# pierric/smart-chess-rust

Measured on AMD Instinct MI355X. Metric: MCTS simulations/sec (whole node), self-play rollout=180, at 1/2/4/8 MI355X, higher is better.
Workload: dtype bf16

## Files before the change

### smart-chess-rust_amd/csrc/mcts_types.hpp

```cpp
#pragma once
#include <stdint.h>

#include "chess_rules.hpp"

namespace sc {

constexpr int MAXC = 224;
enum { ST_IDLE = 0, ST_ACTIVE = 1, ST_FINISHED = 2, ST_PENDING = 3 };
enum { TR_FREE = 0, TR_LIVE = 1, TR_DONE = 2 };
enum { SYNTH_HASH = 1, SYNTH_COARSE = 2, SYNTH_UNIFORM = 3 };
enum { LK_NONE = 0, LK_EVAL = 1, LK_TERM_NEW = 2, LK_TERM_CACHED = 3 };
enum { ERR_NONFINITE_UCT = 1, ERR_POOL_OVERFLOW = 2, ERR_BAD_MOVE_INDEX = 4, ERR_DEPTH_OVERFLOW = 8, ERR_HELPER_TIMEOUT = 16, ERR_HANDOFF_TIMEOUT = 32 };

struct GameCtl {
    int32_t status, ply, sim, n_nodes, n_exp;
    int32_t leaf, path_len, leaf_kind, n_legal;
    float leaf_value;
    uint32_t err;
    int32_t trace_slot;
    uint64_t game_id;
    int32_t start_ply;
    int32_t rollout_cur;
};

struct NodeHdr {
    int32_t fc;
    uint16_t nc;
    uint16_t ps;
};

struct TraceHdr {
    int32_t n_steps, has_outcome, termination, winner;
    uint64_t game_id;
    int32_t state, pad;
};

struct Counters {
    unsigned long long next_game, sims_done, nn_evals, plies_done;
    int32_t games_finished, err;
};

struct SpParams {
    int n_slots, rollout, num_steps, temp_switch, with_noise, outcome_gate, evaluator, external_noise;
    int tie_random;
    int trace_hold;
    float rollout_factor;
    uint64_t synth_salt;
    float cpuct, temperature, epsilon;
    uint64_t seed, first_game_id;
    int node_cap, max_depth, hist_cap, tpos_cap, trace_cap, total_games;
    GameCtl* ctl;
    Position* hist;
    Position* tpos;
    int32_t* path;
    int32_t* N;
    float* W;
    float* P;
    float* U;
    uint16_t* MV;
    NodeHdr* H;
    int8_t* boards;
    int32_t* meta;
    uint16_t* legal_mv;
    uint16_t* legal_idx;
    int32_t* n_legal;
    float* prior;
    float* value;
    float* noise;
    TraceHdr* thdr;
    uint16_t* t_move;
    float* t_q;
    int32_t* t_nchild;
    uint16_t* t_cmove;
    int32_t* t_cn;
    float* t_cq;
    float* t_cu;
    Counters* cnt;
    unsigned long long* slot_cnt;
    int vf_fused, vf_ksplit;
    const float* vpart;
    const float* vf_w;
    uint32_t vf_fc1b, vf_fc1m, vf_fc2w, vf_fc2b;
    const float* choice_w;
    int choice_w_max;
    unsigned long long* dbg_cycles;
};


}
```

### smart-chess-rust_amd/csrc/nn_tower32.hpp

```cpp
#pragma once
#include <type_traits>

#include "nn_kernels.hpp"

namespace scnn {

typedef __attribute__((ext_vector_type(16))) float f32x16;
typedef __attribute__((ext_vector_type(8))) int i32x8;

struct PrecBF16 {
    static constexpr bool FP8 = false;
    static constexpr int EB = 2;
    static constexpr int KS = 16;
    static constexpr int FB = 16;
    typedef bf16x8 frag;
};
struct PrecFP8 {
    static constexpr bool FP8 = true;
    static constexpr int EB = 1;
    static constexpr int KS = 64;
    static constexpr int FB = 32;
    typedef i32x8 frag;
};
template <class P>
// ... 302 lines not shown
    for (int ct = 0; ct < CT; ct++)
#pragma unroll
        for (int pt = 0; pt < 2; pt++)
#pragma unroll
            for (int g = 0; g < 4; g++)
                store4<P, false>(pixbase[pt], chan32<CT>(wave, ct, g, h), pair(acc[ct][pt], 4 * g), pair(acc[ct][pt], 4 * g + 2));
}

template <int CTRL>
__device__ __forceinline__ float dpp_mov(float x) { return dpp_f<CTRL>(x); }
template <int LVL>
__device__ __forceinline__ float pool_xchg(float x) {
    if constexpr (LVL == 1) return dpp_mov<0x140>(x);
    else if constexpr (LVL == 2) return dpp_mov<0x141>(x);
    else if constexpr (LVL == 3) return dpp_mov<0x4E>(x);
    else return dpp_mov<0xB1>(x);
}
template <int NV, int W, int LVL>
__device__ __forceinline__ void pool_level(float (&v)[NV], int lane) {
    if constexpr (LVL < 5) {
        if constexpr (W >= 1) {
            if constexpr (LVL == 0) {
#pragma unroll
                for (int t = 0; t < W; t++) {
                    const auto r = __builtin_amdgcn_permlane16_swap(__float_as_uint(v[t]), __float_as_uint(v[t + W]), false, false);
                    v[t] = __uint_as_float(r[0]) + __uint_as_float(r[1]);
                }
            } else {
                const bool hi = (lane & (16 >> LVL)) != 0;
#pragma unroll
                for (int t = 0; t < W; t++) {
                    float send = hi ? v[t] : v[t + W], keep = hi ? v[t + W] : v[t];
                    v[t] = keep + pool_xchg<LVL>(send);
                }
            }
            pool_level<NV, W / 2, LVL + 1>(v, lane);
        } else {
            v[0] += pool_xchg<LVL>(v[0]);
            pool_level<NV, 0, LVL + 1>(v, lane);
        }
    }
}

template <class P, int CT, int TILES, int RS>
__device__ __forceinline__ void ring_fill(typename P::frag (&bq)[RS][CT], const bf16_t* __restrict__ Wp, int wave_u, int lane) {
    constexpr int TB = 64 * P::FB;
    const __amdgpu_buffer_rsrc_t rsrc = __builtin_amdgcn_make_buffer_rsrc(
        const_cast<bf16_t*>(Wp) + (size_t)wave_u * CT * (TB / 2), 0, 0x7fffffff, 0x00020000);
#pragma unroll
    for (int st = 0; st < RS - 1; st++)
#pragma unroll
        for (int ct = 0; ct < CT; ct++) bq[st][ct] = wload_p<P>(rsrc, lane * 16, ct, st * TILES * TB);
}
template <class P, int CT>
__device__ __forceinline__ void scale_load(int (&sa)[CT], const NetDev& net, int conv_idx, int wave, int lane) {
#pragma unroll
    for (int ct = 0; ct < CT; ct++)
        sa[ct] = P::FP8 ? __builtin_bit_cast(int, net.wf[net.f_scales + (size_t)((conv_idx * 8 + wave * CT + ct) * 64 + lane)]) : 127;
}

constexpr int tower32_lds_bytes(int C, bool fp8 = false) {
    const int psb = C * (fp8 ? 1 : 2) + 16, hpsb = HEAD * (fp8 ? 1 : 2) + 16;
    const int xa = 100 * psb > 4864 * 4 ? 100 * psb : 4864 * 4;
    return xa + 64 * hpsb + 4096 + 3072 + 1024 + 64 + 15 * C * 2;
}

struct NoPre {
    __device__ __forceinline__ bool operator()(int) const { return true; }
};
struct Fc1Hand {
    typedef __attribute__((ext_vector_type(4))) unsigned int u32x4;
    Fc1W w;
    uint32_t early;
    int have_a;
    u32x4 a[8];
};
struct NoHand {};
template <class P, int C, int RS, int TPI, int AB = SC_T32_AB, class Pre = NoPre, class Hand = NoHand>
__device__ __forceinline__ bool tower_body(const TowerArgs& A, const int pos, const int8_t* planes_lds, Pre pre, Hand& fhr) {
    constexpr bool FUSED = !std::is_same<Pre, NoPre>::value;
    constexpr bool HAND = std::is_same<Hand, Fc1Hand>::value;
    Hand* const fh = &fhr;
    typedef typename P::frag frag;
    constexpr int CT = C / 128;
    constexpr int TILES = C / 32;
    constexpr int PSB = pix_stride<P>(C);
    constexpr int HPSB = pix_stride<P>(HEAD);
    constexpr int EB = P::EB;
    constexpr int HRS = P::FP8 ? C / 64 : 8, HAB = P::FP8 ? 2 : SC_T32_AB;
    constexpr int H2RS = P::FP8 ? HEAD / 64 : 16, H2AB = P::FP8 ? 2 : SC_T32_AB;
    constexpr int NTW = C / 64;
    constexpr int XA_BYTES = (100 * PSB > 4864 * 4) ? 100 * PSB : 4864 * 4;
    constexpr int RS_BYTES = 64 * HPSB;
    unsigned char* smem = g_smem;
    float* s_stat = reinterpret_cast<float*>(smem + XA_BYTES + RS_BYTES);
    float* s_vec = s_stat + 1024;
    float* s_scl = s_vec + 768;
    float* s_red = s_scl + 256;
    constexpr int PAR_OFF = XA_BYTES + RS_BYTES + 4096 + 3072 + 1024 + 64;
    bf16_t* s_xb = reinterpret_cast<bf16_t*>(s_vec);
    float* s_z = reinterpret_cast<float*>(smem);
    static_assert(4864 * 4 <= XA_BYTES, "policy logits (and the softmax pass that reads 19 x 256 of them) must fit in the image area");
    static_assert(XA_BYTES % 16 == 0 && RS_BYTES % 16 == 0, "LDS regions must stay 16-byte aligned");

    const int tid = threadIdx.x, lane = tid & 63;
    const int wave = __builtin_amdgcn_readfirstlane(tid >> 6);
    const int i32 = lane & 31, h = lane >> 5;
    const NetDev& net = A.net;
#ifdef SC_EXP
    const bool clk_on = A.dbg && A.dbg_stage == 2001 && tid == 0;
    const long long clk_t0 = clk_on ? clock64() : 0;
    const unsigned long long clk_r0 = clk_on ? __builtin_amdgcn_s_memrealtime() : 0;
    Stamp stampv;
    stampv.on = A.dbg && A.dbg_stage == 2000 && lane == 0;
    stampv.prev = 0;
    for (int k = 0; k < 40; k++) stampv.t[k] = 0;
    stampv.start();
#endif
    const int bp[2] = {gpix2board(0, i32), gpix2board(1, i32)};
    const int pixbase[2] = {hidx(bp[0]) * PSB, hidx(bp[1]) * PSB};
    const int px[2] = {pixbase[0] + h * P::FB, pixbase[1] + h * P::FB};

    frag ring[RS][CT];
    int sa[CT], san[CT];
    scale_load<P, CT>(sa, net, 0, wave, lane);
    scale_load<P, CT>(san, net, net.n_blocks > 0 ? 1 : 1 + 2 * net.n_blocks, wave, lane);
    ChP<CT> Bn;
    constexpr int PAR0 = XA_BYTES + RS_BYTES + 4096 + 3072 + 1024 + 64;
    const int p_in = tid >> 2, q_in = tid & 3;
    uint32_t win[7];
    if (!FUSED && !planes_lds) {
        const uint32_t* src = reinterpret_cast<const uint32_t*>(A.boards + (size_t)pos * 7168 + p_in * 112 + q_in * 28);
#pragma unroll
        for (int k = 0; k < 7; k++) win[k] = src[k];
    }
    static_assert(C <= 256, "one parameter vector per thread");
    f32x4 spv = f32x4{0.f, 0.f, 0.f, 0.f};
    if (tid < 3 * C / 4) spv = *reinterpret_cast<const f32x4*>(net.wf + net.f_stem + tid * 4);
    else if (tid < C) spv = *reinterpret_cast<const f32x4*>(net.wf + net.f_blocks + (tid - 3 * C / 4) * 4);
#ifndef SC_FUSED_RING_LATE
#define SC_FUSED_RING_LATE 1
#endif
    if (!FUSED || wave != 0 || !SC_FUSED_RING_LATE) ring_fill<P, CT, TILES, RS>(ring, net.wb + net.o_stem, wave, lane);
    __builtin_amdgcn_sched_barrier(0);
    if constexpr (FUSED) {
        __shared__ int s_go;
        if (wave <= 1) {
            const bool go = pre(wave);
            if (wave == 0 && lane == 0) s_go = go ? 1 : 0;
            if (wave == 0 && SC_FUSED_RING_LATE) ring_fill<P, CT, TILES, RS>(ring, net.wb + net.o_stem, wave, lane);
        } else {
            uint4* z = reinterpret_cast<uint4*>(smem);
            for (int k = tid - 128; k < 100 * PSB / 16; k += 128) z[k] = make_uint4(0, 0, 0, 0);
        }
        __syncthreads();
        if (!s_go) return false;
    } else {
        uint4* z = reinterpret_cast<uint4*>(smem);
        for (int k = tid; k < 100 * PSB / 16; k += 256) z[k] = make_uint4(0, 0, 0, 0);
        __syncthreads();
    }
    if (FUSED || planes_lds) {
        const uint32_t* src = reinterpret_cast<const uint32_t*>(planes_lds + p_in * 112 + q_in * 28);
#pragma unroll
        for (int k = 0; k < 7; k++) win[k] = src[k];
    }
    {
        uint32_t* dst = reinterpret_cast<uint32_t*>(smem + hidx(p_in) * PSB + q_in * 28 * EB);
#pragma unroll
        for (int k = 0; k < 7; k++) {
            const uint32_t w = win[k];
            float v[4];
#pragma unroll
            for (int b = 0; b < 4; b++) v[b] = (float)(int8_t)((w >> (8 * b)) & 0xff);
            if constexpr (P::FP8) {
                dst[k] = pk_fp8x4(v[0], v[1], v[2], v[3]);
            } else {
                dst[2 * k] = pk_bf16(f32x2{v[0], v[1]});
                dst[2 * k + 1] = pk_bf16(f32x2{v[2], v[3]});
            }
        }
        if (tid < C) *reinterpret_cast<f32x4*>(g_smem + PAR0 + tid * 16) = spv;
    }
    __syncthreads();

    f32x16 acc[CT][2];
    int ln_parity = 0;
    int bad = 0;
    f32x16 res[CT][2];
    auto store_res = [&]() {
#pragma unroll
        for (int ct = 0; ct < CT; ct++)
#pragma unroll
            for (int pt = 0; pt < 2; pt++) res[ct][pt] = acc[ct][pt];
    };
    auto dump = [&](int stage) {
        if constexpr (FUSED) return;
        if (A.dbg && A.dbg_stage == stage) {
#pragma unroll
            for (int ct = 0; ct < CT; ct++)
#pragma unroll
                for (int pt = 0; pt < 2; pt++)
#pragma unroll
                    for (int r = 0; r < 16; r++)
                        A.dbg[((size_t)pos * 64 + bp[pt]) * C + chan32<CT>(wave, ct, r >> 2, h) + (r & 3)] = acc[ct][pt][r];
        }
    };

    SC_MARK(38);
    {
        ch_load_lds<CT>(Bn, PAR0, wave, h);
        acc_init<CT>(acc, Bn);
        const bf16_t* w0 = net.wb + net.o_stem;
        SC_MARK(33);
        conv_mma32<P, 128, 9, CT, TILES, PSB, RS, TPI, true, AB>(0, w0, wave, lane, px, acc, ring, (int)((net.wb + net.o_blocks) - w0) * 2, sa);
        ChP<CT> G, E;
        ch_load_lds<CT>(G, PAR0 + C * 4, wave, h);
        ch_load_lds<CT>(E, PAR0 + 2 * C * 4, wave, h);
        ch_load_lds<CT>(Bn, PAR0 + 3 * C * 4, wave, h);
        SC_MARK(34);
        layernorm32<CT>(acc, G, E, C, true, wave, lane, s_stat, ln_parity, bad SC_STAMP_PASS(35));
        SC_MARK(37);
    }
    store_res();
    store_image32<P, CT>(acc, pixbase, wave, h);
    __syncthreads();
    SC_MARK(14);
    dump(0);
    const int head_conv0 = 1 + 2 * net.n_blocks;

#pragma unroll 1
    for (int b = 0; b < net.n_blocks; b++) {
        const bf16_t* wb = net.wb + net.o_blocks + (size_t)b * net.blk_stride_b;
        const float* wf = net.wf + net.f_blocks + (size_t)b * net.blk_stride_f;
        constexpr int NT1 = C / 32;
        constexpr int NTW1 = NT1 / 4;
        constexpr int PAR_V4 = 15 * C / 8;
        constexpr int NPV = (PAR_V4 + 255) / 256;
        static_assert(PAR0 == PAR_OFF, "prologue staging area");
        constexpr int P_G1 = PAR_OFF, P_E1 = PAR_OFF + 4 * C, P_B2 = PAR_OFF + 8 * C, P_G2 = PAR_OFF + 12 * C, P_E2 = PAR_OFF + 16 * C;
        constexpr int P_SB1 = PAR_OFF + 20 * C, P_SB2 = PAR_OFF + 22 * C, P_BN = PAR_OFF + 26 * C;
#ifdef SC_EXP
        stampv.start();
#endif
        f32x4 pv[NPV];
#pragma unroll
        for (int k = 0; k < NPV; k++)
            if (tid + 256 * k < PAR_V4) pv[k] = *reinterpret_cast<const f32x4*>(wf + C + (size_t)(tid + 256 * k) * 4);
        __builtin_amdgcn_sched_barrier(0);
        acc_init<CT>(acc, Bn);
#pragma unroll
        for (int ct = 0; ct < CT; ct++) sa[ct] = san[ct];
        scale_load<P, CT>(san, net, 2 + 2 * b, wave, lane);
        conv_mma32<P, C, 9, CT, TILES, PSB, RS, TPI, true, AB>(0, wb, wave, lane, px, acc, ring, 9 * C * C * EB, sa);
        SC_MARK(0);
#pragma unroll
        for (int k = 0; k < NPV; k++)
            if (tid + 256 * k < PAR_V4) *reinterpret_cast<f32x4*>(g_smem + PAR_OFF + (tid + 256 * k) * 16) = pv[k];
        {
            LnStat L;
            ln_reduce<CT>(acc, L, C, wave, lane, s_stat, ln_parity, bad SC_STAMP_PASS(1));
            ChP<CT> G, E;
            ch_load_lds<CT>(G, P_G1, wave, h);
            ch_load_lds<CT>(E, P_E1, wave, h);
            SC_MARK(3);
            ln_apply_relu_store<P, CT>(acc, L, G, E, pixbase, wave, h);
        }
        ch_load_lds<CT>(Bn, P_B2, wave, h);
        __syncthreads();
        SC_MARK(4);
        acc_init<CT>(acc, Bn);
        {
            const int nxt = (b + 1 < net.n_blocks) ? (int)(net.blk_stride_b * 2 - (size_t)9 * C * C * EB) : 0;
#pragma unroll
            for (int ct = 0; ct < CT; ct++) sa[ct] = san[ct];
            scale_load<P, CT>(san, net, b + 1 < net.n_blocks ? 3 + 2 * b : head_conv0, wave, lane);
            conv_mma32<P, C, 9, CT, TILES, PSB, RS, TPI, true, AB>(0, wb + (size_t)9 * C * C * EB / 2, wave, lane, px, acc, ring, nxt, sa);
        }
        SC_MARK(5);
        VecW<C, NTW1> w1;
        VecW<C / 2, NTW> w2;
        vec_w_load<C, NTW1, NT1>(w1, wb + (size_t)9 * C * C * EB, wave * NTW1, lane);
        vec_w_load<C / 2, NTW, C / 16>(w2, wb + (size_t)9 * C * C * EB + (size_t)C * (C / 2), wave * NTW, lane);
        __builtin_amdgcn_sched_barrier(0);
        {
            LnStat L;
            ln_reduce<CT>(acc, L, C, wave, lane, s_stat, ln_parity, bad SC_STAMP_PASS(6));
            ChP<CT> G, E;
            ch_load_lds<CT>(G, P_G2, wave, h);
            ch_load_lds<CT>(E, P_E2, wave, h);
            ln_apply<CT>(acc, L, G, E, false);
        }
        SC_MARK(8);
        {
            constexpr int NV = 16 * CT;
            float v[NV];
#pragma unroll
            for (int ct = 0; ct < CT; ct++)
#pragma unroll
                for (int r = 0; r < 16; r += 2) {
                    const f32x2 t = pair(acc[ct][0], r) + pair(acc[ct][1], r);
                    v[ct * 16 + r] = t.x;
                    v[ct * 16 + r + 1] = t.y;
                }
            pool_level<NV, NV / 2, 0>(v, lane);
            const int idx = (NV == 32) ? i32 : (i32 >> 1);
// ... 255 lines not shown
```

### smart-chess-rust_amd/csrc/search_expand.hpp

```cpp
#pragma once
#include "search_select.hpp"
#include "value_tail.hpp"

namespace sc {
__device__ inline void try_start_game(SpParams& p, int g, int lane, unsigned long long k) {
    GameCtl& c = p.ctl[g];
    const int ts = (int)(k % (unsigned long long)p.trace_cap);
    const int st = p.thdr[ts].state;
    const unsigned long long prev_id = p.thdr[ts].game_id;
    bool ok;
    if (k < (unsigned long long)p.trace_cap) ok = st == TR_FREE;
    else ok = prev_id == p.first_game_id + k - (unsigned long long)p.trace_cap && (st == TR_FREE || (st == TR_DONE && !p.trace_hold));
    if (!ok) {
        if (lane == 0) {
            c.status = ST_PENDING;
            c.leaf_kind = LK_NONE;
            c.game_id = p.first_game_id + k;
        }
        return;
    }
    const size_t nb = (size_t)g * p.node_cap;
    if (lane == 0) {
        Position s;
        set_startpos(s);
        s.key = position_key(s);
        p.hist[(size_t)g * p.hist_cap] = s;
        p.tpos[(size_t)g * p.tpos_cap] = s;
        p.N[nb] = 0;
        p.W[nb] = 0.0f;
        p.P[nb] = 0.0f;
        p.U[nb] = 0.0f;
        p.MV[nb] = 0;
        p.H[nb] = NodeHdr{-1, 0, 0};
        c.status = ST_ACTIVE;
        c.ply = 0;
        c.start_ply = 0;
        c.sim = 0;
        c.n_nodes = 1;
        c.n_exp = 1;
        c.leaf = 0;
        c.path_len = 0;
        c.leaf_kind = LK_NONE;
        c.n_legal = 0;
        c.err = 0;
        c.rollout_cur = p.rollout;
        c.game_id = p.first_game_id + k;
        c.trace_slot = ts;
        TraceHdr& th = p.thdr[ts];
        th.n_steps = 0;
        th.has_outcome = 0;
        th.termination = 0;
        th.winner = -1;
        th.game_id = c.game_id;
        th.state = TR_LIVE;
    }
}
__device__ inline void start_new_game(SpParams& p, int g, int lane) {
    GameCtl& c = p.ctl[g];
    unsigned long long k = 0;
    if (lane == 0) k = atomicAdd(&p.cnt->next_game, 1ULL);
    k = __shfl(k, 0, 64);
    if (k >= (unsigned long long)p.total_games) {
        if (lane == 0) {
            c.status = ST_IDLE;
            c.leaf_kind = LK_NONE;
        }
        return;
    }
    try_start_game(p, g, lane, k);
}

__device__ inline void finish_game(SpParams& p, int g, int lane, int has_outcome, int term, int winner) {
    GameCtl& c = p.ctl[g];
    if (lane == 0) {
        TraceHdr& th = p.thdr[c.trace_slot];
        th.n_steps = c.ply - c.start_ply;
        th.has_outcome = has_outcome;
        th.termination = term;
        th.winner = winner;
        th.game_id = c.game_id;
        __threadfence();
        th.state = TR_DONE;
        atomicAdd(&p.cnt->games_finished, 1);
        c.status = ST_FINISHED;
    }
    wave_sync();
    start_new_game(p, g, lane);
}

__device__ inline int choose_child(const int32_t* n_act, int nc, float temperature, float u, int tie_random, int lane, const float* w,
                                   int w_max, float* total) {
    *total = 0.0f;
    if (temperature == 0.0f) {
        int bn = -1, bi = 0x7fffffff;
        for (int i = lane; i < nc; i += 64) {
            int n = n_act[i];
            if (n > bn) {
                bn = n;
                bi = i;
            }
        }
        for (int o = 32; o > 0; o >>= 1) {
            int on = __shfl_xor(bn, o, 64), oi = __shfl_xor(bi, o, 64);
            if (on > bn || (on == bn && oi < bi)) {
                bn = on;
                bi = oi;
            }
        }
        int choice = bi;
        if (tie_random) {
            int cnt = 0;
            for (int i = 0; i < nc; i++) cnt += n_act[i] == bn;
            int k = (int)(u * (float)cnt);
            if (k >= cnt) k = cnt - 1;
            for (int i = 0; i < nc; i++)
                if (n_act[i] == bn && k-- == 0) {
                    choice = i;
                    break;
                }
        }
        return choice;
    }
    const bool plain = 1.0f / temperature == 1.0f;
    auto weight = [&](int n) { return plain ? (float)n : w[n < w_max ? n : w_max]; };
    float sum = 0.0f;
    for (int i = 0; i < nc; i++) sum += weight(n_act[i]);
    *total = sum;
    float x = u * sum;
    float cum = 0.0f;
    int idx = 0;
    for (int i = 0; i < nc - 1; i++) {
        cum += weight(n_act[i]);
        if (cum <= x) idx++;
    }
    return idx;
}

using scvt::ValueTail;
__device__ __forceinline__ void value_tail_issue(const SpParams& p, int g, int lane, ValueTail& t) {
    const float* wf = p.vf_w;
    const int32_t* meta = p.meta + (size_t)g * 8;
#pragma unroll
    for (int k = 0; k < 7; k++) t.meta[k] = meta[k];
    const int j = 2 * lane;
    const float* vp = p.vpart + (size_t)g * 128 + j;
    const size_t vstride = (size_t)p.n_slots * 128;
#pragma unroll
    for (int ks = 0; ks < 32; ks++) t.acc[ks] = *reinterpret_cast<const float2*>(vp + (size_t)ks * vstride);
    if (p.vf_ksplit > 32) {
#pragma unroll
        for (int ks = 32; ks < 64; ks++) t.acc[ks] = *reinterpret_cast<const float2*>(vp + (size_t)ks * vstride);
    } else {
#pragma unroll
        for (int ks = 32; ks < 64; ks++) t.acc[ks] = make_float2(0.f, 0.f);
    }
    t.bias = *reinterpret_cast<const float2*>(wf + p.vf_fc1b + j);
    t.w2 = *reinterpret_cast<const float2*>(wf + p.vf_fc2w + j);
#pragma unroll
    for (int k = 0; k < 7; k++) t.wm[k] = *reinterpret_cast<const float2*>(wf + p.vf_fc1m + k * 128 + j);
    t.fc2b = wf[p.vf_fc2b];
}
__device__ __forceinline__ float value_tail_finish(const SpParams& p, const ValueTail& t) { return scvt::value_tail_compute(t, p.vf_ksplit); }

template <bool SC_ST = true>
__device__ __forceinline__ void dev_expand(SpParams& p, int g, int lane, Position* s_np_p, GameCtl& cs_out, bool& cs_valid) {
#pragma clang fp contract(off)
    Position& s_np = *s_np_p;
    GameCtl& c = p.ctl[g];
    {
        const void *a0 = p.ctl, *a1 = p.path, *a2 = p.prior, *a3 = p.legal_mv, *a4 = p.slot_cnt, *a5 = p.vpart, *a6 = p.vf_w, *a7 = p.meta;
        const int i0 = p.max_depth, i1 = p.vf_fused, i2 = p.n_slots, i3 = p.vf_ksplit;
        const uint32_t u0 = p.vf_fc1b, u1 = p.vf_fc1m, u2 = p.vf_fc2w, u3 = p.vf_fc2b;
        asm volatile("" ::"s"(a0), "s"(a1), "s"(a2), "s"(a3), "s"(a4), "s"(a5), "s"(a6), "s"(a7), "s"(i0), "s"(i1), "s"(i2), "s"(i3), "s"(u0), "s"(u1),
                     "s"(u2), "s"(u3));
    }
    const GameCtl craw = c;
    const int pth_raw = p.path[(size_t)g * p.max_depth + (lane < p.max_depth ? lane : p.max_depth - 1)];
    float prv[4];
    uint16_t lmv[4];
#pragma unroll
    for (int k = 0; k < 4; k++) {
        const int i = lane + 64 * k, ic = i < MAXC ? i : MAXC - 1;
        prv[k] = p.prior[(size_t)g * MAXC + ic];
        lmv[k] = p.legal_mv[(size_t)g * MAXC + ic];
    }
    const unsigned long long sc_sims = p.slot_cnt[(size_t)g * 2], sc_evals = p.slot_cnt[(size_t)g * 2 + 1];
    ValueTail vt;
    if (p.vf_fused) value_tail_issue(p, g, lane, vt);
    __builtin_amdgcn_sched_barrier(0);
    SC_XSTAMP(16);
    const GameCtl cs = uniform(craw);
    SC_XSTAMP(17);
    const int pth = lane < p.max_depth ? pth_raw : 0;
#pragma unroll
    for (int k = 0; k < 4; k++) {
        const int i = lane + 64 * k;
        prv[k] = i < MAXC ? prv[k] : 0.f;
        lmv[k] = i < MAXC ? lmv[k] : (uint16_t)0;
    }
    cs_out = cs;
    cs_valid = true;
    if (cs.status == ST_PENDING) {
        try_start_game(p, g, lane, cs.game_id - p.first_game_id);
        cs_valid = false;
        return;
    }
    if (cs.status != ST_ACTIVE || cs.leaf_kind == LK_NONE) return;
    const size_t nb = (size_t)g * p.node_cap;
    int32_t* N = p.N + nb;
    float* W = p.W + nb;
    float* P = p.P + nb;
    float* U = p.U + nb;
    uint16_t* MV = p.MV + nb;
    NodeHdr* H = p.H + nb;
    const int32_t* path = p.path + (size_t)g * p.max_depth;
    Position* hist = p.hist + (size_t)g * p.hist_cap;
    Position* tpos = p.tpos + (size_t)g * p.tpos_cap;

    const int leaf = cs.leaf, kind = cs.leaf_kind, plen = cs.path_len;
    float value = cs.leaf_value;
    int n_nodes = cs.n_nodes, n_exp = cs.n_exp;
    uint32_t err = 0;
    const bool inpath = lane < plen;
    int n0 = 0;
    float w0 = 0.f;
// ... 143 lines not shown
```

### smart-chess-rust_amd/csrc/search_select.hpp

```cpp
#pragma once
#include <type_traits>
#include <hip/hip_runtime.h>

#include "mcts_types.hpp"
#include "position_chain.hpp"

namespace sc {

using scw::dpp_i, scw::wave_sum_fixed, scw::wave_sum_i;

__device__ __forceinline__ int wave_argmax_last(float u, int idx) {
    unsigned b = __builtin_bit_cast(unsigned, u + 0.0f);
    unsigned key = (b & 0x80000000u) ? ~b : (b | 0x80000000u);
    int hi = idx >= 0 ? (int)key : 0, lo = idx;
    auto step = [&](int ohi, int olo) {
        const bool take = olo >= 0 && (lo < 0 || (unsigned)ohi > (unsigned)hi || ((unsigned)ohi == (unsigned)hi && olo > lo));
        hi = take ? ohi : hi;
        lo = take ? olo : lo;
    };
    step(dpp_i<0xB1>(hi), dpp_i<0xB1>(lo));
    step(dpp_i<0x4E>(hi), dpp_i<0x4E>(lo));
    step(dpp_i<0x141>(hi), dpp_i<0x141>(lo));
    step(dpp_i<0x140>(hi), dpp_i<0x140>(lo));
    int bh = __builtin_amdgcn_readlane(hi, 0), bl = __builtin_amdgcn_readlane(lo, 0);
#pragma unroll
    for (int r = 16; r < 64; r += 16) {
        const int oh = __builtin_amdgcn_readlane(hi, r), ol = __builtin_amdgcn_readlane(lo, r);
        const bool take = ol >= 0 && (bl < 0 || (unsigned)oh > (unsigned)bh || ((unsigned)oh == (unsigned)bh && ol > bl));
        bh = take ? oh : bh;
        bl = take ? ol : bl;
    }
    return bl;
}
__device__ __forceinline__ int wave_argmax_last_lane(float u, bool has) {
    unsigned b = __builtin_bit_cast(unsigned, u + 0.0f);
    unsigned key = (b & 0x80000000u) ? ~b : (b | 0x80000000u);
    int k = has ? (int)key : 0;
    auto umax = [](int a, int b2) { return (int)((unsigned)a > (unsigned)b2 ? (unsigned)a : (unsigned)b2); };
    int m = k;
    m = umax(m, dpp_i<0xB1>(m));
    m = umax(m, dpp_i<0x4E>(m));
    m = umax(m, dpp_i<0x141>(m));
    m = umax(m, dpp_i<0x140>(m));
    const int wm = umax(umax(__builtin_amdgcn_readlane(m, 0), __builtin_amdgcn_readlane(m, 16)),
                        umax(__builtin_amdgcn_readlane(m, 32), __builtin_amdgcn_readlane(m, 48)));
    const unsigned long long mask = __ballot(has && k == wm);
    return mask ? 63 - __clzll((long long)mask) : -1;
}
__device__ __forceinline__ NodeHdr uniform(const NodeHdr& q) {
    NodeHdr r;
    r.fc = uniform(q.fc);
    r.nc = (uint16_t)uniform((int)q.nc);
    r.ps = (uint16_t)uniform((int)q.ps);
    return r;
}
__device__ __forceinline__ GameCtl uniform(const GameCtl& q) {
    GameCtl r;
    r.status = uniform(q.status);
    r.ply = uniform(q.ply);
    r.sim = uniform(q.sim);
    r.n_nodes = uniform(q.n_nodes);
    r.n_exp = uniform(q.n_exp);
    r.leaf = uniform(q.leaf);
    r.path_len = uniform(q.path_len);
    r.leaf_kind = uniform(q.leaf_kind);
    r.n_legal = uniform(q.n_legal);
    r.leaf_value = __builtin_bit_cast(float, uniform(__builtin_bit_cast(int, q.leaf_value)));
    r.err = (uint32_t)uniform((int)q.err);
    r.trace_slot = uniform(q.trace_slot);
    r.game_id = uniform((bb_t)q.game_id);
    r.start_ply = uniform(q.start_ply);
    r.rollout_cur = uniform(q.rollout_cur);
    return r;
}

__device__ inline float u01_open(uint64_t& st) {
#pragma clang fp contract(off)
    st = mix64(st);
    return ((float)(st >> 40) + 0.5f) * (1.0f / 16777216.0f);
}
__device__ inline float gamma03(uint64_t st) {
#pragma clang fp contract(off)
    const float LN2 = 0.69314718f;
    const float alpha = 0.3f;
    const float boost = __builtin_amdgcn_exp2f(__builtin_amdgcn_logf(u01_open(st)) * (1.0f / alpha));
    const float d = alpha + 1.0f - 1.0f / 3.0f;
    const float c = 0.3390317518f;
    for (int it = 0; it < 64; it++) {
        float a = u01_open(st), b = u01_open(st);
        float x = __builtin_amdgcn_sqrtf(-2.0f * LN2 * __builtin_amdgcn_logf(a)) * __builtin_amdgcn_cosf(b);
        float v = 1.0f + c * x;
        if (v <= 0.0f) continue;
        v = v * v * v;
        float u = u01_open(st);
        if (LN2 * __builtin_amdgcn_logf(u) < 0.5f * x * x + d - d * v + d * (LN2 * __builtin_amdgcn_logf(v))) return boost * d * v;
    }
    return boost * d;
}

constexpr int DEPTH_LDS = 1024;

#ifdef SC_EXP
#define SC_XSTAMP(k) SC_STAMP(k)
#else
#define SC_XSTAMP(k)
#endif
#ifdef SC_EXP
#define SC_ST_DEFAULT true
#else
#define SC_ST_DEFAULT false
#endif
#define SC_STAMP(k)                                                                       \
    do {                                                                                  \
        if constexpr (SC_ST) {                                                            \
            if (p.dbg_cycles && lane == 0) p.dbg_cycles[(size_t)g * 32 + (k)] = clock64(); \
        }                                                                                 \
    } while (0)

struct HelperBox {
    int state, idx, root_ply, pad;
};
__device__ __forceinline__ void helper_post(HelperBox* box, int lane, int state, int idx, int root_ply) {
    if (!box) return;
    if (lane == 0) {
        box->idx = idx;
        box->root_ply = root_ply;
    }
    wave_sync();
    if (lane == 0) *reinterpret_cast<volatile int*>(&box->state) = state;
}
__device__ __forceinline__ void dev_encode_helper(const SpParams& p, int g, int lane, HelperBox* box, int8_t* s_stage, Position* s_leaf_p,
                                                  uint16_t* s_ps, Position* s_hist) {
    int st = 0;
    for (int spin = 0; spin < (1 << 22) && st == 0; spin++) {
        st = *reinterpret_cast<volatile int*>(&box->state);
        if (st == 0) __builtin_amdgcn_s_sleep(2);
    }
    st = __builtin_amdgcn_readfirstlane(st);
    if (st == 0 && lane == 0) atomicOr(&p.cnt->err, ERR_HELPER_TIMEOUT);
    if (st != 1 && st != 3) return;
    wave_sync();
    const int idx = __builtin_amdgcn_readfirstlane(box->idx), root_ply = __builtin_amdgcn_readfirstlane(box->root_ply);
    DevChain ch{p.hist + (size_t)g * p.hist_cap, root_ply, p.tpos + (size_t)g * p.tpos_cap, s_ps, s_leaf_p, idx};
    if (st == 3) {
        const bb_t key0 = s_leaf_p->key;
        const uint8_t rf = (uint8_t)__builtin_amdgcn_readfirstlane((int)rep_flags_wave(ch, idx, key0, lane));
        const uint8_t fl = (uint8_t)((s_leaf_p->flags & F_IRREV) | rf);
        wave_sync();
        if (lane == 0) {
            s_leaf_p->flags = fl;
            box->pad = fl;
        }
        wave_sync();
        if (lane == 0) *reinterpret_cast<volatile int*>(&box->state) = 4;
    }
    stage_history(ch, idx, lane, s_hist);
    wave_sync();
    encode_wave(s_hist, idx < 7 ? idx + 1 : 8, lane, s_stage, nullptr, p.meta + (size_t)g * 8);
}

template <bool PLANES_TO_HBM = true, bool SC_ST = true>
__device__ __forceinline__ bool dev_select(const SpParams& p, int g, int lane, int8_t* s_stage, move_t* s_moves, Position* s_leaf_p,
                                        uint16_t* s_ps, Position* s_hist, const GameCtl& cs_pre, bool cs_pre_valid,
                                        HelperBox* box = nullptr) {
#pragma clang fp contract(off)
    Position& s_leaf = *s_leaf_p;
    SC_STAMP(2);
    GameCtl& c = p.ctl[g];
    GameCtl cs = cs_pre;
    if (!cs_pre_valid) cs = uniform(c);
    const Position root_raw = p.tpos[(size_t)g * p.tpos_cap];
    const NodeHdr hdr_raw = p.H[(size_t)g * p.node_cap];
    const size_t nb0 = (size_t)g * p.node_cap + (1 + lane < p.node_cap ? 1 + lane : p.node_cap - 1);
    const int pf_n = p.N[nb0];
    const float pf_w = p.W[nb0], pf_p = p.P[nb0];
    const NodeHdr pf_h = p.H[nb0];
    __builtin_amdgcn_sched_barrier(0);
    const Position root = uniform(root_raw);
    NodeHdr hdr = uniform(hdr_raw);
    if (cs.status != ST_ACTIVE) {
        if (lane == 0) c.leaf_kind = LK_NONE;
        helper_post(box, lane, 2, 0, 0);
        return false;
    }
    const size_t nb = (size_t)g * p.node_cap;
    const int32_t* N = p.N + nb;
    const float* W = p.W + nb;
    const float* P = p.P + nb;
    float* U = p.U + nb;
    const uint16_t* MV = p.MV + nb;
    const NodeHdr* H = p.H + nb;
    int32_t* path = p.path + (size_t)g * p.max_depth;
    const Position* hist = p.hist + (size_t)g * p.hist_cap;
    Position* tpos = p.tpos + (size_t)g * p.tpos_cap;
    const int root_ply = cs.ply;
    const int root_turn = root.turn;
    const int dmax = p.max_depth < DEPTH_LDS ? p.max_depth : DEPTH_LDS;

    int node = 0, depth = 0, parent_ps = 0;
    if (lane == 0) {
        path[0] = 0;
        s_ps[0] = 0;
    }
    uint32_t err = 0;
    for (;;) {
        const int nc = hdr.nc;
        if (nc == 0) break;
        const int fc = hdr.fc;
        const int nr = (nc + 63) >> 6;
        int best_i = 0;
        NodeHdr nxt;
        auto level = [&](auto nrc) {
#pragma clang fp contract(off)
            constexpr int NRM = decltype(nrc)::value;
            int cn[NRM];
            float cw[NRM], cp[NRM];
            NodeHdr ch_[NRM];
#pragma unroll
            for (int r = 0; r < NRM; r++) {
                cn[r] = 0;
                cw[r] = 0.f;
                cp[r] = 0.f;
                ch_[r] = NodeHdr{-1, 0, 0};
                if (r < nr) {
                    int i = lane + 64 * r;
                    bool ok = i < nc;
                    if (r == 0 && depth == 0 && fc == 1) {
                        cn[0] = ok ? pf_n : 0;
                        cw[0] = ok ? pf_w : 0.f;
                        cp[0] = ok ? pf_p : 0.f;
                        ch_[0] = ok ? pf_h : NodeHdr{-1, 0, 0};
                    } else {
                        cn[r] = ok ? N[fc + i] : 0;
                        cw[r] = ok ? W[fc + i] : 0.f;
                        cp[r] = ok ? P[fc + i] : 0.f;
                        ch_[r] = ok ? H[fc + i] : NodeHdr{-1, 0, 0};
                    }
                }
            }
            if (nc > 1) {
                const bool reverse_q = ((root_turn ^ (depth & 1)) == BLACK);
                const bool noisy = depth == 0 && p.with_noise;
                float* nz = p.noise + (size_t)g * MAXC;
                float nzv[NRM];
#pragma unroll
                for (int r = 0; r < NRM; r++) nzv[r] = 0.f;
                if (noisy) {
                    if (!p.external_noise) {
                        float gsum = 0.0f;
#pragma unroll
                        for (int r = 0; r < NRM; r++) {
                            int i = lane + 64 * r;
                            if (i < nc) {
                                nzv[r] = gamma03(sc_rng(p.seed, cs.game_id, (uint64_t)root_ply, 3, (uint64_t)cs.sim * 256 + (uint64_t)i));
                                gsum += nzv[r];
                            }
                        }
                        gsum = wave_sum_fixed(gsum);
#pragma unroll
                        for (int r = 0; r < NRM; r++) {
                            int i = lane + 64 * r;
                            nzv[r] = nzv[r] / gsum;
                            if (i < nc) nz[i] = nzv[r];
                        }
                    } else {
#pragma unroll
                        for (int r = 0; r < NRM; r++) {
                            int i = lane + 64 * r;
                            if (i < nc) nzv[r] = nz[i];
                        }
                    }
                }
                int tot = 0;
#pragma unroll
                for (int r = 0; r < NRM; r++) tot += cn[r];
                tot = wave_sum_i(tot);
                const float sqrt_total = sqrtf((float)tot);
                float best_u = 0.0f;
                best_i = -1;
#pragma unroll
                for (int r = 0; r < NRM; r++) {
                    int i = lane + 64 * r;
                    if (r < nr && i < nc) {
                        float prior = cp[r];
                        if (noisy) prior = prior * (1.0f - p.epsilon) + nzv[r] * p.epsilon;
                        float average_award = cw[r] / ((float)cn[r] + 1e-4f) * (reverse_q ? -1.0f : 1.0f);
                        float exploration = (sqrt_total + 0.01f) / (1.0f + (float)cn[r]) * p.cpuct * prior;
                        float u = average_award + exploration;
                        U[fc + i] = u;
                        if (!isfinite(u)) err |= ERR_NONFINITE_UCT;
                        if (best_i < 0 || u >= best_u) {
                            best_u = u;
                            best_i = i;
                        }
                    }
                }
                if constexpr (NRM == 1) best_i = wave_argmax_last_lane(best_u, best_i >= 0);
                else best_i = wave_argmax_last(best_u, best_i);
            }
            best_i = __builtin_amdgcn_readfirstlane(best_i);
            const int rr = best_i >> 6;
            NodeHdr mine = ch_[0];
#pragma unroll
            for (int r = 1; r < NRM; r++)
                if (rr == r) mine = ch_[r];
            nxt.fc = __builtin_amdgcn_readlane(mine.fc, best_i & 63);
            int packed = __builtin_amdgcn_readlane((int)mine.nc | ((int)mine.ps << 16), best_i & 63);
            nxt.nc = (uint16_t)(packed & 0xffff);
            nxt.ps = (uint16_t)((unsigned)packed >> 16);
        };
        if (nr == 1) level(std::integral_constant<int, 1>{});
        else level(std::integral_constant<int, 4>{});
        parent_ps = hdr.ps;
        node = fc + best_i;
        hdr = nxt;
        depth++;
        if (depth >= dmax) {
            err |= ERR_DEPTH_OVERFLOW;
            depth--;
            break;
        }
        if (lane == 0) {
            path[depth] = node;
            s_ps[depth] = hdr.ps;
        }
    }
    SC_STAMP(3);
    if (p.dbg_cycles && lane == 0) p.dbg_cycles[(size_t)g * 32 + 7] = depth;
    unsigned long long anyerr = __ballot(err != 0);
    if (anyerr) {
        for (int o = 32; o > 0; o >>= 1) err |= __shfl_xor(err, o, 64);
        if (lane == 0) {
            c.err = cs.err | err;
            atomicOr(&p.cnt->err, (int)err);
        }
    }
    const int fcl = hdr.fc;
    if (lane == 0) {
        c.leaf = node;
        c.path_len = depth + 1;
    }
    if (fcl <= -2) {
        if (lane == 0) {
            c.leaf_kind = LK_TERM_CACHED;
            c.leaf_value = fcl == -2 ? 0.0f : fcl == -3 ? 1.0f : -1.0f;
            c.n_legal = 0;
        }
        helper_post(box, lane, 2, 0, 0);
        return false;
    }
    Position pos;
    if (depth == 0) {
        pos = root;
    } else {
        pos = uniform(tpos[parent_ps]);
        make_move(pos, (move_t)__builtin_amdgcn_readfirstlane((int)MV[node]));
    }
    if (lane == 0) s_leaf = pos;
    wave_sync();
    DevChain ch{hist, root_ply, tpos, s_ps, &s_leaf, root_ply + depth};
    const bool rep_by_helper = box && depth > 0;
    if (depth > 0 && !box) {
        uint8_t rf = (uint8_t)__builtin_amdgcn_readfirstlane((int)rep_flags_wave(ch, root_ply + depth, pos.key, lane));
        pos.flags = (uint8_t)((pos.flags & F_IRREV) | rf);
        wave_sync();
        if (lane == 0) s_leaf.flags = pos.flags;
        wave_sync();
    }
    SC_STAMP(4);
    if (box) helper_post(box, lane, rep_by_helper ? 3 : 1, root_ply + depth, root_ply);
    else stage_history(ch, root_ply + depth, lane, s_hist);
    if (lane == 0 && !rep_by_helper) tpos[cs.n_exp] = pos;
    int n = 0;
    bool in_check = gen_legal_wave(pos, s_moves, lane, n);
    wave_sync();
    SC_STAMP(5);
    if (depth == 0 && p.rollout_factor > 0.f && lane == 0) {
        const int r = (int)((float)n * p.rollout_factor);
        c.rollout_cur = r < 300 ? r : 300;
    }
    if (n == 0) {
        if (lane == 0) {
            c.leaf_kind = LK_TERM_NEW;
            c.leaf_value = in_check ? (pos.turn == WHITE ? -1.0f : 1.0f) : 0.0f;
            c.n_legal = 0;
        }
        return false;
    }
    uint16_t* lm = p.legal_mv + (size_t)g * MAXC;
    uint16_t* li = p.legal_idx + (size_t)g * MAXC;
    uint32_t bad = 0;
    for (int i = lane; i < n; i += 64) {
        move_t m = s_moves[i];
        int idx = move_index(m, pos.turn);
        if (idx < 0) {
            bad = 1;
            idx = 0;
        }
        lm[i] = m;
        li[i] = (uint16_t)idx;
    }
    if (__ballot(bad) && lane == 0) {
        c.err = cs.err | err | ERR_BAD_MOVE_INDEX;
        atomicOr(&p.cnt->err, ERR_BAD_MOVE_INDEX);
    }
    if (rep_by_helper) {
        int st = 3;
        for (int spin = 0; spin < (1 << 22) && st != 4; spin++) {
            st = *reinterpret_cast<volatile int*>(&box->state);
            if (st != 4) __builtin_amdgcn_s_sleep(1);
        }
        st = __builtin_amdgcn_readfirstlane(st);
        wave_sync();
        if (st != 4 && lane == 0) atomicOr(&p.cnt->err, ERR_HELPER_TIMEOUT);
        pos.flags = (uint8_t)__builtin_amdgcn_readfirstlane(box->pad);
        if (lane == 0) tpos[cs.n_exp] = pos;
    }
    const int idx = root_ply + depth;
// ... 12 lines not shown
```

### smart-chess-rust_amd/csrc/step_kernels.hip

```cpp
#include "search_expand.hpp"
#include "nn_kernels.hpp"
#include "nn_tower32.hpp"

#include "launchers.hpp"
#include "tower_config.hpp"

namespace scstep {

__device__ __forceinline__ void fc1_tail(const scnn::TowerArgs& A, const sc::SpParams& p, const int g, const bool ran, scnn::Fc1Hand& fh) {
    const int tid = threadIdx.x, lane = tid & 63;
    const int wave = __builtin_amdgcn_readfirstlane(tid >> 6);
    const int mb = g >> 6, ks = g & 63;
    uint32_t* ctr = A.fc1_arrive + mb * 32;
#ifdef SC_EXP
#define TSTAMP(k) do { if (p.dbg_cycles && tid == 0) p.dbg_cycles[(size_t)g * 32 + 8 + (k)] = __builtin_amdgcn_s_memrealtime(); } while (0)
#else
#define TSTAMP(k)
#endif
    TSTAMP(0);
    if (!ran) {
        if (tid == 0) __hip_atomic_fetch_add(ctr, 1u, __ATOMIC_RELAXED, __HIP_MEMORY_SCOPE_AGENT);
        scnn::fc1_wload(fh.w, A.net, ks, 64, wave, lane);
        __builtin_amdgcn_sched_barrier(0);
    }
    const scnn::Fc1W& w = fh.w;
    const bool have_a = ran && fh.have_a;
#ifdef SC_EXP
    if (p.dbg_cycles && tid == 0) p.dbg_cycles[(size_t)g * 32 + 14] = have_a;
    if (have_a) { TSTAMP(1); TSTAMP(2); }
#endif
    if (tid == 0 && !have_a) {
        const uint64_t t0 = __builtin_amdgcn_s_memrealtime();
        uint32_t seen = ran ? fh.early : __hip_atomic_load(ctr, __ATOMIC_RELAXED, __HIP_MEMORY_SCOPE_AGENT);
        while ((int32_t)(seen - A.fc1_target) < 0) {
            __builtin_amdgcn_s_sleep(4);
            const uint64_t waited = __builtin_amdgcn_s_memrealtime() - t0;
            if (waited > 20000000ull) {
                atomicOr(&p.cnt->err, sc::ERR_HANDOFF_TIMEOUT);
                break;
            }
            if (waited > 100000ull && (__hip_atomic_load(&p.cnt->err, __ATOMIC_RELAXED, __HIP_MEMORY_SCOPE_AGENT) & sc::ERR_HANDOFF_TIMEOUT)) break;
            seen = __hip_atomic_load(ctr, __ATOMIC_RELAXED, __HIP_MEMORY_SCOPE_AGENT);
        }
        TSTAMP(1);
        if (A.fc1_acquire) __builtin_amdgcn_fence(__ATOMIC_ACQUIRE, "agent");
        asm volatile("s_waitcnt vmcnt(0)" ::: "memory");
        TSTAMP(2);
    }
    __syncthreads();
    scnn::bf16_t* s_a = reinterpret_cast<scnn::bf16_t*>(scnn::g_smem);
    if (!have_a) scnn::fc1_load_a(fh.a, A.hval, mb, ks, tid);
    scnn::fc1_put_a(s_a, fh.a, tid);
    __syncthreads();
    TSTAMP(3);
    scnn::fc1_mma_store(w, s_a, A.vpart, A.n_pos, mb, ks, 64, wave, lane);
    TSTAMP(4);
#ifdef SC_EXP
    asm volatile("s_waitcnt vmcnt(0)" ::: "memory");
    TSTAMP(5);
#endif
}

template <class P, int C, int RS, int TPI, int AB, bool STAMPS = false>
__global__ __launch_bounds__(256, 1) void k_step(scnn::TowerArgs A, sc::SpParams p, int do_expand) {
    __shared__ __attribute__((aligned(16))) int8_t s_stage[7168];
    __shared__ sc::move_t s_moves[sc::MAXC];
    __shared__ sc::Position s_pos;
    __shared__ sc::Position s_hist[8];
    __shared__ uint16_t s_ps[sc::DEPTH_LDS];
    __shared__ sc::HelperBox s_box;
    const int g = blockIdx.x;
    const int lane = threadIdx.x & 63;
#ifdef SC_EXP
    const long long t_entry = clock64();
#endif
    scnn::kernarg_prefetch<sizeof(scnn::TowerArgs) + sizeof(sc::SpParams) + sizeof(int)>();
#ifdef SC_EXP
    if (p.dbg_cycles && threadIdx.x == 0) p.dbg_cycles[(size_t)g * 32 + 21] = t_entry;
#endif
#define PHASE_STAMP(k, cond) do { if constexpr (STAMPS) { if (p.dbg_cycles && (cond)) p.dbg_cycles[(size_t)g * 32 + (k)] = __builtin_amdgcn_s_memrealtime(); } } while (0)
    PHASE_STAMP(24, threadIdx.x == 0);
    if (threadIdx.x == 0) s_box.state = 0;
    __syncthreads();
    auto search = [&](int wave) -> bool {
        if (wave == 1) {
            sc::dev_encode_helper(p, g, lane, &s_box, s_stage, &s_pos, s_ps, s_hist);
            return true;
        }
        constexpr bool SC_ST = STAMPS || SC_ST_DEFAULT;
        SC_STAMP(0);
        sc::GameCtl cs_pre{};
        bool cs_pre_valid = false;
        if (do_expand) {
            sc::dev_expand<SC_ST>(p, g, lane, &s_pos, cs_pre, cs_pre_valid);
            __builtin_amdgcn_wave_barrier();
        }
        SC_STAMP(1);
        const bool need_net = sc::dev_select<false, SC_ST>(p, g, lane, s_stage, s_moves, &s_pos, s_ps, s_hist, cs_pre, cs_pre_valid, &s_box);
        PHASE_STAMP(25, lane == 0);
        return need_net;
    };
    scnn::Fc1Hand fh;
    const bool ran = scnn::tower_body<P, C, RS, TPI, AB>(A, g, s_stage, search, fh);
    PHASE_STAMP(26, threadIdx.x == 0);
    if (A.fc1_arrive) fc1_tail(A, p, g, ran, fh);
    PHASE_STAMP(27, threadIdx.x == 0);
#undef PHASE_STAMP
}

}

namespace scl {
#define K_STEP(P, C, RS, TPI, AB) scstep::k_step<scnn::P, C, RS, TPI, AB>
#define K_STEP_STAMPED scstep::k_step<scnn::PrecBF16, 128, SC_T32_RS, SC_T32_TPI, SC_T32_AB, true>
const char* step_init() {
    const void* kn[4] = {reinterpret_cast<const void*>(&K_STEP(PrecBF16, 128, SC_T32_RS, SC_T32_TPI, SC_T32_AB)),
                         reinterpret_cast<const void*>(&K_STEP(PrecBF16, 256, SC_T32W_RS, SC_T32W_TPI, SC_T32W_AB)),
                         reinterpret_cast<const void*>(&K_STEP(PrecFP8, 128, SC_T8_RS, SC_T8_TPI, SC_T8_AB)),
                         reinterpret_cast<const void*>(&K_STEP(PrecFP8, 256, SC_T8W_RS, SC_T8W_TPI, SC_T8W_AB))};
    for (int i = 0; i < 4; i++) {
        hipError_t e = hipFuncSetAttribute(kn[i], hipFuncAttributeMaxDynamicSharedMemorySize, scnn::tower32_lds_bytes(i & 1 ? 256 : 128, i >= 2 && i < 4));
        if (e != hipSuccess) return hipGetErrorString(e);
    }
    {
        hipError_t e = hipFuncSetAttribute(reinterpret_cast<const void*>(&K_STEP_STAMPED), hipFuncAttributeMaxDynamicSharedMemorySize, scnn::tower32_lds_bytes(128));
        if (e != hipSuccess) return hipGetErrorString(e);
    }
    return nullptr;
}
int step_blocks_per_cu(const scnn::NetLayout& net) {
    int n = 0;
    hipError_t e;
    if (net.fp8 && net.C == 128)
        e = hipOccupancyMaxActiveBlocksPerMultiprocessor(&n, K_STEP(PrecFP8, 128, SC_T8_RS, SC_T8_TPI, SC_T8_AB), 256, scnn::tower32_lds_bytes(128, true));
    else if (net.fp8)
        e = hipOccupancyMaxActiveBlocksPerMultiprocessor(&n, K_STEP(PrecFP8, 256, SC_T8W_RS, SC_T8W_TPI, SC_T8W_AB), 256, scnn::tower32_lds_bytes(256, true));
    else if (net.C == 128)
        e = hipOccupancyMaxActiveBlocksPerMultiprocessor(&n, K_STEP(PrecBF16, 128, SC_T32_RS, SC_T32_TPI, SC_T32_AB), 256, scnn::tower32_lds_bytes(128));
    else
        e = hipOccupancyMaxActiveBlocksPerMultiprocessor(&n, K_STEP(PrecBF16, 256, SC_T32W_RS, SC_T32W_TPI, SC_T32W_AB), 256, scnn::tower32_lds_bytes(256));
    return e == hipSuccess && n > 0 ? n : 1;
}
void step(const scnn::TowerArgs& a, const sc::SpParams& p, int do_expand, hipStream_t s) {
    const dim3 grid(p.n_slots), block(256);
    if (a.net.fp8 && a.net.C == 128)
        hipLaunchKernelGGL((K_STEP(PrecFP8, 128, SC_T8_RS, SC_T8_TPI, SC_T8_AB)), grid, block, scnn::tower32_lds_bytes(128, true), s, a, p, do_expand);
    else if (a.net.fp8)
        hipLaunchKernelGGL((K_STEP(PrecFP8, 256, SC_T8W_RS, SC_T8W_TPI, SC_T8W_AB)), grid, block, scnn::tower32_lds_bytes(256, true), s, a, p, do_expand);
    else if (a.net.C == 128 && p.dbg_cycles)
        hipLaunchKernelGGL((K_STEP_STAMPED), grid, block, scnn::tower32_lds_bytes(128), s, a, p, do_expand);
    else if (a.net.C == 128)
        hipLaunchKernelGGL((K_STEP(PrecBF16, 128, SC_T32_RS, SC_T32_TPI, SC_T32_AB)), grid, block, scnn::tower32_lds_bytes(128), s, a, p, do_expand);
    else
        hipLaunchKernelGGL((K_STEP(PrecBF16, 256, SC_T32W_RS, SC_T32W_TPI, SC_T32W_AB)), grid, block, scnn::tower32_lds_bytes(256), s, a, p, do_expand);
}
}
```

Before: 2.256 million.

## Offload root Dirichlet noise generation to a helper wave in the fused step

Adds a helper routine run by wave 2 inside the fused tower prologue. It precomputes the root Dirichlet noise (gamma samples, then normalisation) into LDS and publishes the result through a shared NoiseBox. The selecting wave spins on the box, checks that ply, sim, child count and game id match, and then reuses the values, falling back to computing the noise itself otherwise. The aim is to take gamma sampling off wave 0's select critical path, at the cost of extra LDS, a spin-wait with a timeout, and the helper's own global reads.

```diff
diff --git a/smart-chess-rust_amd/csrc/mcts_types.hpp b/smart-chess-rust_amd/csrc/mcts_types.hpp
--- a/smart-chess-rust_amd/csrc/mcts_types.hpp
+++ b/smart-chess-rust_amd/csrc/mcts_types.hpp
@@ -10,6 +10,7 @@
 enum { TR_FREE = 0, TR_LIVE = 1, TR_DONE = 2 };
 enum { SYNTH_HASH = 1, SYNTH_COARSE = 2, SYNTH_UNIFORM = 3 };
 enum { LK_NONE = 0, LK_EVAL = 1, LK_TERM_NEW = 2, LK_TERM_CACHED = 3 };
+enum { DBG_NOISE_USED = 28, DBG_NOISE_WAIT = 29 };
 enum { ERR_NONFINITE_UCT = 1, ERR_POOL_OVERFLOW = 2, ERR_BAD_MOVE_INDEX = 4, ERR_DEPTH_OVERFLOW = 8, ERR_HELPER_TIMEOUT = 16, ERR_HANDOFF_TIMEOUT = 32 };
 
 struct GameCtl {
diff --git a/smart-chess-rust_amd/csrc/nn_tower32.hpp b/smart-chess-rust_amd/csrc/nn_tower32.hpp
--- a/smart-chess-rust_amd/csrc/nn_tower32.hpp
+++ b/smart-chess-rust_amd/csrc/nn_tower32.hpp
@@ -478,6 +478,7 @@
         } else {
             uint4* z = reinterpret_cast<uint4*>(smem);
             for (int k = tid - 128; k < 100 * PSB / 16; k += 128) z[k] = make_uint4(0, 0, 0, 0);
+            if (wave == 2) pre(2);
         }
         __syncthreads();
         if (!s_go) return false;
diff --git a/smart-chess-rust_amd/csrc/search_expand.hpp b/smart-chess-rust_amd/csrc/search_expand.hpp
--- a/smart-chess-rust_amd/csrc/search_expand.hpp
+++ b/smart-chess-rust_amd/csrc/search_expand.hpp
@@ -70,7 +70,7 @@
     try_start_game(p, g, lane, k);
 }
 
-__device__ inline void finish_game(SpParams& p, int g, int lane, int has_outcome, int term, int winner) {
+__device__ __forceinline__ void finish_game(SpParams& p, int g, int lane, int has_outcome, int term, int winner) {
     GameCtl& c = p.ctl[g];
     if (lane == 0) {
         TraceHdr& th = p.thdr[c.trace_slot];
diff --git a/smart-chess-rust_amd/csrc/search_select.hpp b/smart-chess-rust_amd/csrc/search_select.hpp
--- a/smart-chess-rust_amd/csrc/search_select.hpp
+++ b/smart-chess-rust_amd/csrc/search_select.hpp
@@ -159,13 +159,58 @@
     encode_wave(s_hist, idx < 7 ? idx + 1 : 8, lane, s_stage, nullptr, p.meta + (size_t)g * 8);
 }
 
+struct NoiseBox {
+    int state;
+    int ply, sim, nc;
+    uint64_t game_id;
+};
+__device__ __forceinline__ void dev_noise_helper(const SpParams& p, int g, int lane, int do_expand, NoiseBox* nbox, float* s_noise) {
+#pragma clang fp contract(off)
+    int state = 2;
+    if (p.with_noise && !p.external_noise) {
+        const GameCtl craw = p.ctl[g];
+        const NodeHdr hraw = p.H[(size_t)g * p.node_cap];
+        __builtin_amdgcn_sched_barrier(0);
+        const GameCtl cs = uniform(craw);
+        const NodeHdr h0 = uniform(hraw);
+        const bool pending = do_expand && cs.leaf_kind != LK_NONE;
+        const int sim = cs.sim + (pending ? 1 : 0);
+        const int budget = p.rollout_factor > 0.f ? cs.rollout_cur : p.rollout;
+        const int nc = pending && cs.leaf_kind == LK_EVAL && cs.leaf == 0 ? cs.n_legal : (int)h0.nc;
+        if (cs.status == ST_ACTIVE && !(pending && sim >= budget) && nc > 1 && nc <= MAXC) {
+            float gsum = 0.0f;
+#pragma unroll 1
+            for (int i = lane; i < nc; i += 64) {
+                const float v = gamma03(sc_rng(p.seed, cs.game_id, (uint64_t)cs.ply, 3, (uint64_t)sim * 256 + (uint64_t)i));
+                s_noise[i] = v;
+                gsum += v;
+            }
+            gsum = wave_sum_fixed(gsum);
+#pragma unroll 1
+            for (int i = lane; i < nc; i += 64) s_noise[i] = s_noise[i] / gsum;
+            if (lane == 0) {
+                nbox->ply = cs.ply;
+                nbox->sim = sim;
+                nbox->nc = nc;
+                nbox->game_id = cs.game_id;
+            }
+            state = 1;
+        }
+    }
+    wave_sync();
+    if (lane == 0) *reinterpret_cast<volatile int*>(&nbox->state) = state;
+}
+
 template <bool PLANES_TO_HBM = true, bool SC_ST = true>
 __device__ __forceinline__ bool dev_select(const SpParams& p, int g, int lane, int8_t* s_stage, move_t* s_moves, Position* s_leaf_p,
                                         uint16_t* s_ps, Position* s_hist, const GameCtl& cs_pre, bool cs_pre_valid,
-                                        HelperBox* box = nullptr) {
+                                        HelperBox* box = nullptr, NoiseBox* nbox = nullptr, const float* s_noise = nullptr) {
 #pragma clang fp contract(off)
     Position& s_leaf = *s_leaf_p;
     SC_STAMP(2);
+    if constexpr (SC_ST) {
+        if (p.dbg_cycles && lane == 0) p.dbg_cycles[(size_t)g * 32 + DBG_NOISE_USED] = p.dbg_cycles[(size_t)g * 32 + DBG_NOISE_WAIT] = 0;
+    }
     GameCtl& c = p.ctl[g];
     GameCtl cs = cs_pre;
     if (!cs_pre_valid) cs = uniform(c);
@@ -246,7 +291,39 @@
 #pragma unroll
                 for (int r = 0; r < NRM; r++) nzv[r] = 0.f;
                 if (noisy) {
-                    if (!p.external_noise) {
+                    bool helped = false;
+                    if (nbox && !p.external_noise) {
+                        long long t0 = 0;
+                        if constexpr (SC_ST) t0 = clock64();
+                        int st = 0;
+                        for (int spin = 0; spin < (1 << 22) && st == 0; spin++) {
+                            st = *reinterpret_cast<volatile int*>(&nbox->state);
+                            if (st == 0) __builtin_amdgcn_s_sleep(1);
+                        }
+                        st = __builtin_amdgcn_readfirstlane(st);
+                        if (st == 0 && lane == 0) atomicOr(&p.cnt->err, ERR_HELPER_TIMEOUT);
+                        const volatile NoiseBox* vb = nbox;
+                        helped = st == 1 && uniform(vb->ply) == root_ply && uniform(vb->sim) == cs.sim && uniform(vb->nc) == nc &&
+                                 uniform((uint64_t)vb->game_id) == cs.game_id;
+                        if (helped) {
+                            const volatile float* vn = s_noise;
+#pragma unroll
+                            for (int r = 0; r < NRM; r++) {
+                                int i = lane + 64 * r;
+                                if (i < nc) {
+                                    nzv[r] = vn[i];
+                                    nz[i] = nzv[r];
+                                }
+                            }
+                        }
+                        if constexpr (SC_ST) {
+                            if (p.dbg_cycles && lane == 0) {
+                                p.dbg_cycles[(size_t)g * 32 + DBG_NOISE_USED] = helped;
+                                p.dbg_cycles[(size_t)g * 32 + DBG_NOISE_WAIT] = clock64() - t0;
+                            }
+                        }
+                    }
+                    if (!p.external_noise && !helped) {
                         float gsum = 0.0f;
 #pragma unroll
                         for (int r = 0; r < NRM; r++) {
@@ -263,7 +340,7 @@
                             nzv[r] = nzv[r] / gsum;
                             if (i < nc) nz[i] = nzv[r];
                         }
-                    } else {
+                    } else if (p.external_noise) {
 #pragma unroll
                         for (int r = 0; r < NRM; r++) {
                             int i = lane + 64 * r;
diff --git a/smart-chess-rust_amd/csrc/step_kernels.hip b/smart-chess-rust_amd/csrc/step_kernels.hip
--- a/smart-chess-rust_amd/csrc/step_kernels.hip
+++ b/smart-chess-rust_amd/csrc/step_kernels.hip
@@ -69,6 +69,8 @@
     __shared__ sc::Position s_hist[8];
     __shared__ uint16_t s_ps[sc::DEPTH_LDS];
     __shared__ sc::HelperBox s_box;
+    __shared__ sc::NoiseBox s_nbox;
+    __shared__ float s_noise[sc::MAXC];
     const int g = blockIdx.x;
     const int lane = threadIdx.x & 63;
 #ifdef SC_EXP
@@ -80,11 +82,18 @@
 #endif
 #define PHASE_STAMP(k, cond) do { if constexpr (STAMPS) { if (p.dbg_cycles && (cond)) p.dbg_cycles[(size_t)g * 32 + (k)] = __builtin_amdgcn_s_memrealtime(); } } while (0)
     PHASE_STAMP(24, threadIdx.x == 0);
-    if (threadIdx.x == 0) s_box.state = 0;
+    if (threadIdx.x == 0) {
+        s_box.state = 0;
+        s_nbox.state = 0;
+    }
     __syncthreads();
     auto search = [&](int wave) -> bool {
         if (wave == 1) {
             sc::dev_encode_helper(p, g, lane, &s_box, s_stage, &s_pos, s_ps, s_hist);
+            return true;
+        }
+        if (wave == 2) {
+            sc::dev_noise_helper(p, g, lane, do_expand, &s_nbox, s_noise);
             return true;
         }
         constexpr bool SC_ST = STAMPS || SC_ST_DEFAULT;
@@ -96,7 +105,7 @@
             __builtin_amdgcn_wave_barrier();
         }
         SC_STAMP(1);
-        const bool need_net = sc::dev_select<false, SC_ST>(p, g, lane, s_stage, s_moves, &s_pos, s_ps, s_hist, cs_pre, cs_pre_valid, &s_box);
+        const bool need_net = sc::dev_select<false, SC_ST>(p, g, lane, s_stage, s_moves, &s_pos, s_ps, s_hist, cs_pre, cs_pre_valid, &s_box, &s_nbox, s_noise);
         PHASE_STAMP(25, lane == 0);
         return need_net;
     };
```

After: 2.232 million. -1.1%, worse.
